# ambonvik/cimba

Measured on NVIDIA H100. Metric: M/M/1 simulated events/sec (FEL pops/s), higher is better.
Workload: dtype f64

## Files before the change

cimba_b200/_lib.py:

```python
from __future__ import annotations

import ctypes as C
from pathlib import Path

import os

LIB_PATH = Path(os.environ.get("CIMBA_B200_LIB") or
                Path(__file__).resolve().parent / "lib" / "libcimba_b200.so")

NO_FIELD = C.c_size_t(-1).value

MODEL_MM1, MODEL_GG1, MODEL_MMC, MODEL_GUARDED, MODEL_PREEMPT, MODEL_BUFFER, MODEL_PRIOQ, MODEL_HOLD, MODEL_TIMERS, MODEL_MM1_RECORDED, MODEL_HARBOR, MODEL_GUARDED_RECORDED, MODEL_BUFFER_RECORDED, MODEL_PRIOQ_RECORDED, MODEL_RESOURCE_RECORDED, MODEL_AWACS = 0, 1, 2, 3, 4, 5, 6, 7, 8, 9, 10, 11, 12, 13, 14, 15
MODEL_RENEGE, MODEL_POOL_RECORDED, MODEL_TUTORIAL1, MODEL_PARK, MODEL_TUTORIAL2, MODEL_USER_BASE, VARIANT_GENERAL, VARIANT_STATIC = 16, 18, 19, 20, 21, 1000, 16, 17
MAP_LANE, MAP_WARP = 1, 32

OK, EINVAL, ENODEVICE, ECUDA, ETRIAL, ENOMEM = 0, -1, -2, -3, -4, -5


class DeviceJob(C.Structure):
    _fields_ = [
        ("model", C.c_int32), ("servers", C.c_int32), ("mapping", C.c_int32), ("variant", C.c_int32),
        ("master_seed", C.c_uint64), ("first_trial", C.c_uint64),
        ("num_trials", C.c_uint64), ("num_objects", C.c_uint64),
        ("arr_mean", C.c_void_p), ("srv_mean", C.c_void_p),
        ("events", C.c_void_p), ("objects", C.c_void_p),
        ("t_end", C.c_void_p), ("sum_wait", C.c_void_p),
        ("status", C.c_void_p), ("max_queue", C.c_void_p), ("counters", C.c_void_p),
        ("workspace", C.c_void_p), ("workspace_bytes", C.c_uint64),
        ("trace_cap", C.c_uint64), ("trace_key", C.c_void_p), ("trace_time", C.c_void_p),
        ("queue_spill_cap", C.c_uint32), ("reserved0", C.c_uint32), ("diag", C.c_void_p),
        ("params", C.POINTER(C.c_double)), ("num_params", C.c_uint32), ("reserved1", C.c_uint32),
    ]


class AwacsTerrain(C.Structure):
    _fields_ = [("map", C.c_void_p), ("cols", C.c_uint32), ("rows", C.c_uint32),
                ("x_scale", C.c_float), ("y_scale", C.c_float),
                ("x_min", C.c_float), ("x_max", C.c_float), ("y_min", C.c_float), ("y_max", C.c_float)]


THREAD_INIT_FUNC = C.CFUNCTYPE(C.c_void_p, C.c_void_p, C.c_uint64)
THREAD_EXIT_FUNC = C.CFUNCTYPE(None, C.c_void_p)


class Experiment(C.Structure):
    _fields_ = [
        ("model", C.c_int32), ("servers", C.c_int32), ("mapping", C.c_int32), ("device", C.c_int32),
        ("variant", C.c_int32), ("queue_spill_cap", C.c_uint32),
        ("master_seed", C.c_uint64), ("first_trial", C.c_uint64), ("num_objects", C.c_uint64),
        ("off_arr_mean", C.c_size_t), ("off_srv_mean", C.c_size_t),
        ("off_obj_cnt", C.c_size_t), ("off_sum_wait", C.c_size_t), ("off_avg_wait", C.c_size_t),
        ("off_events", C.c_size_t), ("off_t_end", C.c_size_t), ("off_status", C.c_size_t),
        ("off_max_queue", C.c_size_t), ("off_counters", C.c_size_t),
        ("params", C.POINTER(C.c_double)), ("num_params", C.c_uint32), ("reserved", C.c_uint32),
    ]


class DataSummaryStruct(C.Structure):
    _fields_ = [
        ("cookie", C.c_uint64), ("count", C.c_uint64),
        ("min", C.c_double), ("max", C.c_double),
        ("m1", C.c_double), ("m2", C.c_double), ("m3", C.c_double), ("m4", C.c_double),
    ]


class WtdSummaryStruct(C.Structure):
    _fields_ = [("base", DataSummaryStruct), ("wsum", C.c_double)]


SYMBOLS = {
    "cimba_b200_workspace_bytes": (C.c_uint64, [C.POINTER(DeviceJob)]),
    "cimba_b200_launch": (C.c_int, [C.POINTER(DeviceJob), C.c_void_p]),
    "cimba_b200_launch_count": (C.c_uint64, []),
    "cimba_b200_summarize": (C.c_int, [C.c_void_p, C.c_void_p, C.c_uint64, C.c_void_p, C.c_void_p]),
    "cimba_b200_run_experiment": (C.c_int, [C.c_void_p, C.c_uint64, C.c_size_t, C.POINTER(Experiment)]),
    "cimba_b200_release_cache": (None, []),
    "cimba_b200_run_experiment_all_gpus": (C.c_int, [C.c_void_p, C.c_uint64, C.c_size_t, C.POINTER(Experiment),
                                                     C.c_int]),
    "cimba_b200_awacs_set_terrain": (C.c_int, [C.POINTER(AwacsTerrain)]),
    "cimba_b200_awacs_upload_terrain": (C.c_int, [C.POINTER(AwacsTerrain)]),
    "cimba_b200_set_thread_hooks": (None, [C.c_void_p, C.c_void_p, C.c_void_p]),
    "cimba_b200_thread_context": (C.c_void_p, []),
    "cimba_b200_datasummary_initialize": (None, [C.POINTER(DataSummaryStruct)]),
    "cimba_b200_datasummary_add": (C.c_uint64, [C.POINTER(DataSummaryStruct), C.c_double]),
    "cimba_b200_datasummary_merge": (C.c_uint64, [C.POINTER(DataSummaryStruct)] * 3),
    "cimba_b200_datasummary_mean": (C.c_double, [C.POINTER(DataSummaryStruct)]),
    "cimba_b200_datasummary_variance": (C.c_double, [C.POINTER(DataSummaryStruct)]),
    "cimba_b200_datasummary_stddev": (C.c_double, [C.POINTER(DataSummaryStruct)]),
    "cimba_b200_datasummary_count": (C.c_uint64, [C.POINTER(DataSummaryStruct)]),
    "cimba_b200_datasummary_max": (C.c_double, [C.POINTER(DataSummaryStruct)]),
    "cimba_b200_datasummary_min": (C.c_double, [C.POINTER(DataSummaryStruct)]),
    "cimba_b200_datasummary_skewness": (C.c_double, [C.POINTER(DataSummaryStruct)]),
    "cimba_b200_datasummary_kurtosis": (C.c_double, [C.POINTER(DataSummaryStruct)]),
    "cimba_b200_datasummary_print": (None, [C.POINTER(DataSummaryStruct), C.c_void_p, C.c_int]),
    "cimba_b200_summarize_weighted": (C.c_int, [C.c_void_p, C.c_void_p, C.c_uint64, C.c_void_p, C.c_void_p]),
    "cimba_b200_merge_weighted_rows": (C.c_int, [C.c_void_p, C.c_uint64, C.c_void_p, C.c_void_p]),
    "cimba_b200_wtdsummary_initialize": (None, [C.POINTER(WtdSummaryStruct)]),
    "cimba_b200_wtdsummary_add": (C.c_uint64, [C.POINTER(WtdSummaryStruct), C.c_double, C.c_double]),
    "cimba_b200_wtdsummary_merge": (C.c_uint64, [C.POINTER(WtdSummaryStruct)] * 3),
    "cimba_b200_wtdsummary_mean": (C.c_double, [C.POINTER(WtdSummaryStruct)]),
    "cimba_b200_wtdsummary_variance": (C.c_double, [C.POINTER(WtdSummaryStruct)]),
    "cimba_b200_wtdsummary_stddev": (C.c_double, [C.POINTER(WtdSummaryStruct)]),
    "cimba_b200_wtdsummary_skewness": (C.c_double, [C.POINTER(WtdSummaryStruct)]),
    "cimba_b200_wtdsummary_kurtosis": (C.c_double, [C.POINTER(WtdSummaryStruct)]),
    "cimba_b200_wtdsummary_print": (None, [C.POINTER(WtdSummaryStruct), C.c_void_p, C.c_int]),
    "cimba_b200_fmix64": (C.c_uint64, [C.c_uint64, C.c_uint64]),
    "cimba_b200_rng_draws": (C.c_int, [C.c_uint64, C.c_int, C.c_double, C.c_double,
                                       C.c_uint64, C.c_void_p, C.c_void_p]),
    "cimba_b200_rng_draws_ex": (C.c_int, [C.c_uint64, C.c_int, C.POINTER(C.c_double), C.c_uint32,
                                          C.c_uint64, C.c_void_p, C.c_void_p]),
    "cimba_b200_alias_create": (C.c_int, [C.c_uint32, C.POINTER(C.c_double), C.POINTER(C.c_uint64),
                                          C.POINTER(C.c_uint32)]),
    "cimba_b200_model_load": (C.c_int, [C.c_char_p]),
    "cimba_b200_model_name": (C.c_char_p, [C.c_int]),
    "cimba_b200_version": (C.c_char_p, []),
    "cimba_b200_last_error": (C.c_char_p, []),
    "cimba_b200_device_count": (C.c_int, []),
}


def load() -> C.CDLL:
    if not LIB_PATH.exists():
        raise ImportError(
            f"{LIB_PATH} is missing: build it with `python -c 'import __graft_entry__ as g; g.build()'` "
            "(nvcc, sm_90a). cimba_b200 has no CPU fallback.")
    lib = C.CDLL(str(LIB_PATH))
    for name, (res, args) in SYMBOLS.items():
        fn = getattr(lib, name)
        fn.restype = res
        fn.argtypes = args
    return lib


lib = load()


class CimbaError(RuntimeError):
    def __init__(self, code: int):
        self.code = code
        msg = lib.cimba_b200_last_error().decode(errors="replace")
        super().__init__(f"cimba_b200 error {code}: {msg}")


def check(code: int) -> None:
    if code != OK:
        raise CimbaError(code)
```

cimba_b200/csrc/capi.cu:

```cuda
#include <atomic>
#include <chrono>
#include <cfloat>
#include <cmath>
#include <cstdio>
#include <cstdlib>
#include <cstring>
#include <deque>
#include <mutex>
#include <string>
#include <thread>
#include <vector>

#include <cuda_runtime.h>

#include "../../include/cimba_b200.h"
#include "engine.cuh"
#include "queue_model.cuh"
#include "mm1_fast.cuh"
#include "mm1_pc.cuh"
#include "gg1_fast.cuh"
#include "pool_model.cuh"
#include "pool_fast.cuh"
#include "guarded_model.cuh"
#include "preempt_model.cuh"
// ... 257 lines not shown
}

template <class Model>
uint64_t engine_workspace(const cimba_b200_device_job *job) { return cmb::workspace_bytes_for<Model>(*job); }

int engine_checks(const cimba_b200_device_job *job, const char *servers_msg)
{
    if (mapping_of(job) != CIMBA_B200_MAP_LANE) return fail(CIMBA_B200_EINVAL, "the general engine runs one trial per lane (CIMBA_B200_MAP_LANE)");
    if (servers_msg != nullptr && job->servers < 1) return fail(CIMBA_B200_EINVAL, servers_msg);
    return check_workspace(job);
}

template <class Model>
int launch_engine(const cimba_b200_device_job *job, cudaStream_t st, const char *what)
{
    return counted(cmb::launch_model<Model>(*job, (unsigned char *)job->workspace, job->workspace_bytes, 0u, st), what);
}

template <class Model> const char *const ENGINE_WHAT = nullptr;
template <> const char *const ENGINE_WHAT<models::MM1> = "trial_kernel<MM1> launch";
template <> const char *const ENGINE_WHAT<models::GG1> = "trial_kernel<GG1> launch";
template <> const char *const ENGINE_WHAT<models::MM1Recorded> = "trial_kernel<MM1Recorded> launch";
template <> const char *const ENGINE_WHAT<models::MMC> = "trial_kernel<MMC> launch";
template <> const char *const ENGINE_WHAT<models::HoldGeneral> = "trial_kernel<HoldGeneral> launch";
template <> const char *const ENGINE_WHAT<models::Renege> = "trial_kernel<Renege> launch";
template <> const char *const ENGINE_WHAT<models::Cheese> = "trial_kernel<Cheese> launch";
template <> const char *const ENGINE_WHAT<models::Tutorial1> = "trial_kernel<Tutorial1> launch";
template <> const char *const ENGINE_WHAT<models::Park> = "trial_kernel<Park> launch";
template <> const char *const ENGINE_WHAT<models::Tutorial2> = "trial_kernel<Tutorial2> launch";

template <class Model>
int engine_launch(const cimba_b200_device_job *job, cudaStream_t st)
{
    if (const int e = engine_checks(job, "servers must be >= 1")) return e;
    return launch_engine<Model>(job, st, ENGINE_WHAT<Model>);
}

template <class Model>
constexpr Route ENGINE{engine_workspace<Model>, engine_launch<Model>};

int harbor_engine_launch(const cimba_b200_device_job *job, cudaStream_t st)
{
    if (const int e = engine_checks(job, "servers must be >= 1")) return e;
    if (job->servers < 3) return fail(CIMBA_B200_EINVAL, "tugs (servers) must be >= 3 for CIMBA_B200_MODEL_HARBOR (a large ship needs 3)");
    return launch_engine<models::HarborGeneral>(job, st, "trial_kernel<HarborGeneral> launch");
}

template <template <class> class ModelT, int NPROC, int NQUEUE, int NEVENT = 0>
uint64_t static_workspace(const cimba_b200_device_job *job) { return cmb::workspace_bytes_static<ModelT, NPROC, NQUEUE, NEVENT>(*job); }

template <template <class> class ModelT, int NPROC, int NQUEUE, int NEVENT = 0>
int static_launch(const cimba_b200_device_job *job, cudaStream_t st)
{
    if (mapping_of(job) != CIMBA_B200_MAP_LANE) return fail(CIMBA_B200_EINVAL, "the static tier runs one trial per lane (CIMBA_B200_MAP_LANE)");
    if (const int e = check_workspace(job)) return e;
    return counted(cmb::launch_static_model<ModelT, NPROC, NQUEUE, NEVENT>(*job, st), "static_trial_kernel launch",
                   job->status != nullptr ? 2 : 1);
}

template <template <class> class ModelT, int NPROC, int NQUEUE, int NEVENT = 0>
constexpr Route STATIC{static_workspace<ModelT, NPROC, NQUEUE, NEVENT>, static_launch<ModelT, NPROC, NQUEUE, NEVENT>};

template <template <class> class ModelT, int NPROC, int NEVENT, uint64_t (*WORKSPACE)(const cimba_b200_device_job *), bool SERVERS>
int static_launch_in(const cimba_b200_device_job *job, cudaStream_t st)
{
    if (mapping_of(job) != CIMBA_B200_MAP_LANE) return fail(CIMBA_B200_EINVAL, "the static tier runs one trial per lane (CIMBA_B200_MAP_LANE)");
    if (SERVERS && job->servers < 1) return fail(CIMBA_B200_EINVAL, "servers must be >= 1");
    if (const int e = check_workspace(job)) return e;
    return counted(cmb::launch_static_trials<ModelT, NPROC, 0, NEVENT>(*job, st), "static_trial_kernel launch",
                   job->status != nullptr ? 2 : 1);
}

template <template <class> class ModelT, int NPROC, int NEVENT, uint64_t (*WORKSPACE)(const cimba_b200_device_job *), bool SERVERS>
constexpr Route STATIC_IN{WORKSPACE, static_launch_in<ModelT, NPROC, NEVENT, WORKSPACE, SERVERS>};

uint64_t queue_rings_bytes(const cimba_b200_device_job *job)
{
    const uint32_t cap = cmb::spill_cap(*job);
    return job->num_trials * (uint64_t)(cap == 0u ? cmb::SPILL_CAP_DEFAULT : cap) * sizeof(double);
}

uint64_t queue_workspace(const cimba_b200_device_job *job) { return cmb::rings_then_arena(queue_rings_bytes(job), repair_arena_bytes(job)); }

int queue_launch(const cimba_b200_device_job *job, cudaStream_t st)
{
    if (const int e = check_workspace(job)) return e;
    const int mapping = mapping_of(job);
    QueueArgs qa = cmb::job_args<QueueArgs>(*job);
    qa.mapping = mapping;
    qa.num_objects = job->num_objects;
    qa.arr_mean = job->arr_mean;
    qa.srv_mean = job->srv_mean;
    qa.counters = job->counters;
    qa.spill = (double *)job->workspace;
    qa.spill_cap = cmb::spill_cap(*job);
    qa.diag = (unsigned long long *)job->diag;
    const uint64_t threads = job->num_trials * (uint64_t)mapping;
    const uint64_t blocks = (threads + QUEUE_BLOCK - 1) / QUEUE_BLOCK;
    if (blocks > 0x7fffffffull) return fail(CIMBA_B200_EINVAL, "too many trials for one launch");
    const dim3 grid((unsigned)blocks);
    const uint64_t rings = queue_rings_bytes(job);
    if (job->model == CIMBA_B200_MODEL_GG1) {
        if (job->variant == 1) return launch_kernel(job, queue_kernel<1, false>, queue_kernel<1, true>, grid, QUEUE_BLOCK, 0, st, qa, "queue_kernel launch");
        return then_repair<models::GG1>(launch_kernel(job, gg1_kernel<false>, gg1_kernel<true>, grid, QUEUE_BLOCK, 0, st, qa, "gg1_kernel launch"),
                                        job, rings, st, "repair pass (G/G/1)");
    }
    if (job->model == CIMBA_B200_MODEL_MM1_RECORDED) {
        if (job->counters == nullptr)
            return fail(CIMBA_B200_EINVAL, "CIMBA_B200_MODEL_MM1_RECORDED writes its cmb_wtdsummary to counters[]");
        const int e = launch_kernel(job, queue_kernel<0, false, true>, queue_kernel<0, true, true>, grid, QUEUE_BLOCK, 0, st, qa,
                                    "queue_kernel (recorded) launch");
        return then_repair<models::MM1Recorded>(e, job, rings, st, "repair pass (M/M/1 with its queue history)");
    }
    if (job->variant == 1) return launch_kernel(job, queue_kernel<0, false>, queue_kernel<0, true>, grid, QUEUE_BLOCK, 0, st, qa, "queue_kernel launch");
    int e;
    if (job->variant == 2) {
        if (mapping != CIMBA_B200_MAP_LANE) return fail(CIMBA_B200_EINVAL, "variant 2 of MODEL_MM1 runs one trial per lane");
        const dim3 pc_grid((unsigned)((job->num_trials + MM1_PC_CONSUMERS - 1) / MM1_PC_CONSUMERS));
        e = launch_kernel(job, mm1_pc_kernel<false>, mm1_pc_kernel<true>, pc_grid, 2 * MM1_PC_CONSUMERS, 0, st, qa, "mm1_kernel launch");
    }
    else {
        e = launch_kernel(job, mm1_kernel<false>, mm1_kernel<true>, grid, QUEUE_BLOCK, 0, st, qa, "mm1_kernel launch");
    }
    return then_repair<models::MM1>(e, job, rings, st, "repair pass (M/M/1)");
}

int mmc_launch(const cimba_b200_device_job *job, cudaStream_t st)
{
    if (job->servers < 1) return fail(CIMBA_B200_EINVAL, "servers must be >= 1 for CIMBA_B200_MODEL_MMC");
    if (mapping_of(job) != CIMBA_B200_MAP_LANE) return fail(CIMBA_B200_EINVAL, "MODEL_MMC supports CIMBA_B200_MAP_LANE only");
    if (const int e = check_workspace(job)) return e;
    PoolArgs pa = cmb::job_args<PoolArgs>(*job);
    pa.servers = job->servers;
    pa.num_objects = job->num_objects;
    pa.arr_mean = job->arr_mean;
    pa.srv_mean = job->srv_mean;
    pa.spill = (double *)job->workspace;
    pa.spill_cap = cmb::spill_cap(*job);
    pa.diag = (unsigned long long *)job->diag;
    const uint64_t blocks = (job->num_trials + POOL_BLOCK - 1) / POOL_BLOCK;
    if (blocks > 0x7fffffffull) return fail(CIMBA_B200_EINVAL, "too many trials for one launch");
    const bool readable = job->variant == 1;
    const int e = launch_kernel(job, readable ? pool_kernel<false> : pool_fast_kernel<false>, readable ? pool_kernel<true> : pool_fast_kernel<true>,
                                dim3((unsigned)blocks), POOL_BLOCK, 0, st, pa, "pool_kernel launch");
    return then_repair<models::MMC>(e, job, queue_rings_bytes(job), st, "repair pass (M/M/c)");
}

bool has_capacity(const cimba_b200_device_job *job)
{
    return job->model != CIMBA_B200_MODEL_TIMERS && job->model != CIMBA_B200_MODEL_RESOURCE_RECORDED;
}

template <bool TRACE>
auto coverage_kernel(int m)
{
    return m == CIMBA_B200_MODEL_RESOURCE_RECORDED ? resource_kernel<TRACE>
         : m == CIMBA_B200_MODEL_TIMERS ? timers_kernel<TRACE>
         : m == CIMBA_B200_MODEL_PRIOQ ? prioq_kernel<TRACE>
         : m == CIMBA_B200_MODEL_BUFFER || m == CIMBA_B200_MODEL_BUFFER_RECORDED ? buffer_kernel<TRACE>
         : m == CIMBA_B200_MODEL_PREEMPT ? preempt_kernel<TRACE>
                                         : guarded_kernel<TRACE>;
}

uint64_t coverage_workspace(const cimba_b200_device_job *job)
{
    return cmb::rings_then_arena(job->num_trials * (uint64_t)sizeof(GeneralState), repair_arena_bytes(job));
}

template <class Model>
int coverage_launch(const cimba_b200_device_job *job, cudaStream_t st)
{
    const int m = job->model;
    if (has_capacity(job) && job->servers < 1) return fail(CIMBA_B200_EINVAL, "capacity (servers) must be >= 1");
    if (mapping_of(job) != CIMBA_B200_MAP_LANE) return fail(CIMBA_B200_EINVAL, "MODEL_GUARDED supports CIMBA_B200_MAP_LANE only");
    if (const int e = check_workspace(job)) return e;
    GuardedArgs ga = cmb::job_args<GuardedArgs>(*job);
    ga.capacity = job->servers;
    ga.duration = job->num_objects;
    ga.put_mean = job->arr_mean;
    ga.get_mean = job->srv_mean;
    ga.counters = job->counters;
    ga.state = (GeneralState *)job->workspace;
    ga.record = (m == CIMBA_B200_MODEL_GUARDED_RECORDED || m == CIMBA_B200_MODEL_BUFFER_RECORDED || m == CIMBA_B200_MODEL_PRIOQ_RECORDED) ? 1u : 0u;
    ga.use_pq = m == CIMBA_B200_MODEL_PRIOQ_RECORDED ? 1u : 0u;
    const uint64_t blocks = (job->num_trials + GUARDED_BLOCK - 1) / GUARDED_BLOCK;
    if (blocks > 0x7fffffffull) return fail(CIMBA_B200_EINVAL, "too many trials for one launch");
    const int e = launch_kernel(job, coverage_kernel<false>(m), coverage_kernel<true>(m), dim3((unsigned)blocks), GUARDED_BLOCK, 0, st, ga,
                                "guarded_kernel launch");
    return then_repair<Model>(e, job, job->num_trials * (uint64_t)sizeof(GeneralState), st, "repair pass");
}

template <class Model>
int coverage_engine_launch(const cimba_b200_device_job *job, cudaStream_t st)
{
    if (const int e = engine_checks(job, has_capacity(job) ? "capacity (servers) must be >= 1" : nullptr)) return e;
    return launch_engine<Model>(job, st, "trial_kernel launch");
}

template <class Model>
const Route *coverage_route(const cimba_b200_device_job *job, int max_servers)
{
    static constexpr Route fast{coverage_workspace, coverage_launch<Model>};
    static constexpr Route engine{engine_workspace<Model>, coverage_engine_launch<Model>};
    return job->variant == CIMBA_B200_VARIANT_GENERAL || job->servers > max_servers ? &engine : &fast;
// ... 107 lines not shown
        const int lanes = job->variant == 2 ? 32 : (job->variant == 4 ? 8 : (job->variant == 3 ? 16 : HOLD_DEFAULT_LANES));
        const void *fn = trace ? (const void *)deep_kernel<true>(lanes) : (const void *)deep_kernel<false>(lanes);
        const uint64_t trials_per_block = (uint64_t)(DEEP_BLOCK / 32) * (uint64_t)(32 / lanes);
        if (const int e = resident_grid(fn, DEEP_BLOCK, 0, 8, (job->num_trials + trials_per_block - 1) / trials_per_block, &blocks)) return e;
        DeepArgs da{};
        da.h = ha;
        da.rows = (uint4 *)job->workspace;
        da.row_entries = deep_row_entries(job->servers);
        return launch_kernel(job, deep_kernel<false>(lanes), deep_kernel<true>(lanes), dim3(blocks), DEEP_BLOCK, 0, st, da, "hold_deep_kernel launch");
    }
    const void *fn = trace ? (const void *)hold_kernel<true> : (const void *)hold_kernel<false>;
    if (const int e = resident_grid(fn, 32, HOLD_SMEM_BYTES, 8, job->num_trials, &blocks)) return e;
    return launch_kernel(job, hold_kernel<false>, hold_kernel<true>, dim3(blocks), 32, HOLD_SMEM_BYTES, st, ha, "hold_kernel launch");
}

uint64_t user_workspace(const cimba_b200_device_job *job) { return user_model(job->model)->workspace_bytes(job); }

int user_launch(const cimba_b200_device_job *job, cudaStream_t st)
{
    if (const int e = check_workspace(job)) return e;
    const UserModel *um = user_model(job->model);
    return counted(um->launch(job, st), um->name.c_str());
}

constexpr Route QUEUE{queue_workspace, queue_launch};
constexpr Route MMC_FAST{queue_workspace, mmc_launch};
constexpr Route HARBOR{harbor_workspace, harbor_launch};
constexpr Route HARBOR_ENGINE{engine_workspace<models::HarborGeneral>, harbor_engine_launch};
constexpr Route AWACS{awacs_workspace, awacs_launch};
constexpr Route HOLD{hold_workspace, hold_launch};
constexpr Route USER{user_workspace, user_launch};

const Route *route(const cimba_b200_device_job *job)
{
    const bool general = job->variant == CIMBA_B200_VARIANT_GENERAL, on_static = job->variant == CIMBA_B200_VARIANT_STATIC;
    switch (job->model) {
    case CIMBA_B200_MODEL_MM1:          return on_static ? &STATIC<models::MM1T, 2, 1> : general ? &ENGINE<models::MM1> : &QUEUE;
    case CIMBA_B200_MODEL_GG1:          return on_static ? &STATIC<models::GG1T, 2, 1> : general ? &ENGINE<models::GG1> : &QUEUE;
    case CIMBA_B200_MODEL_MM1_RECORDED: return on_static ? &STATIC<models::MM1RecordedT, 2, 1> : general ? &ENGINE<models::MM1Recorded> : &QUEUE;
    case CIMBA_B200_MODEL_TUTORIAL1:    return general ? &ENGINE<models::Tutorial1> : &STATIC<models::Tutorial1T, 2, 0, 3>;
    case CIMBA_B200_MODEL_MMC:          return general || job->servers > 14 ? &ENGINE<models::MMC> : &MMC_FAST;
    case CIMBA_B200_MODEL_HOLD:         return general ? &ENGINE<models::HoldGeneral> : &HOLD;
    case CIMBA_B200_MODEL_HARBOR:       return general ? &HARBOR_ENGINE : &HARBOR;
    case CIMBA_B200_MODEL_AWACS:        return &AWACS;
    case CIMBA_B200_MODEL_RENEGE:       return &ENGINE<models::Renege>;
    case CIMBA_B200_MODEL_POOL_RECORDED:
        return on_static ? &STATIC_IN<models::CheeseT, 6, 6, engine_workspace<models::Cheese>, true> : &ENGINE<models::Cheese>;
    case CIMBA_B200_MODEL_PARK:         return &ENGINE<models::Park>;
    case CIMBA_B200_MODEL_TUTORIAL2:
        return on_static ? &STATIC_IN<models::Tutorial2T, 8, 8, engine_workspace<models::Tutorial2>, true> : &ENGINE<models::Tutorial2>;
    case CIMBA_B200_MODEL_GUARDED:
        return on_static ? &STATIC_COVERAGE<models::GuardedQueueT, 7, 1, 2, 16> : coverage_route<models::Guarded<false, false>>(job, 16);
    case CIMBA_B200_MODEL_GUARDED_RECORDED:
        return on_static ? &STATIC_COVERAGE<models::GuardedRecordedQueueT, 7, 1, 2, 16> : coverage_route<models::Guarded<false, true>>(job, 16);
    case CIMBA_B200_MODEL_PRIOQ_RECORDED:
        return on_static ? &STATIC_COVERAGE<models::GuardedPriorityQueueT, 7, 0, 2, 15> : coverage_route<models::Guarded<true, true>>(job, 15);
    case CIMBA_B200_MODEL_PRIOQ:
        return on_static ? &STATIC_COVERAGE<models::QueueAndTideT, 8, 0, 2, 15> : coverage_route<models::QueueAndTide>(job, 15);
    case CIMBA_B200_MODEL_PREEMPT:
        return on_static ? &STATIC_IN<models::PoolFightT, 6, models::POOLFIGHT_SPARE_SLOTS, coverage_workspace, true>
                         : coverage_route<models::PoolFight>(job, INT32_MAX);
    case CIMBA_B200_MODEL_BUFFER:
        return on_static ? &STATIC_IN<models::WorkshopBufferT, 7, models::WORKSHOP_SPARE_SLOTS, coverage_workspace, true>
                         : coverage_route<models::Workshop<false>>(job, INT32_MAX);
    case CIMBA_B200_MODEL_BUFFER_RECORDED:
        return on_static ? &STATIC_IN<models::WorkshopRecordedT, 7, models::WORKSHOP_SPARE_SLOTS, coverage_workspace, true>
                         : coverage_route<models::Workshop<true>>(job, INT32_MAX);
    case CIMBA_B200_MODEL_TIMERS:
        return on_static ? &STATIC_IN<models::FrontDeskT, 8, models::FRONTDESK_SPARE_SLOTS, coverage_workspace, false>
                         : coverage_route<models::FrontDesk>(job, INT32_MAX);
    case CIMBA_B200_MODEL_RESOURCE_RECORDED:
        return on_static ? &STATIC_IN<models::ToolT, 4, 2, coverage_workspace, false> : coverage_route<models::Tool>(job, INT32_MAX);
    }
    return job->model >= CIMBA_B200_MODEL_USER_BASE && user_model(job->model) != nullptr ? &USER : nullptr;
}

}

extern "C" {

const char *cimba_b200_version(void) { return CIMBA_B200_VERSION_STRING; }
const char *cimba_b200_last_error(void) { return g_err; }
uint64_t cimba_b200_launch_count(void) { return g_launches.load(); }
uint64_t cimba_b200_fmix64(uint64_t seed, uint64_t nonce) { return fmix64(seed, nonce); }

int cimba_b200_device_count(void)
{
    int n = 0;
    if (cudaGetDeviceCount(&n) != cudaSuccess) {
        (void)cudaGetLastError();
        return 0;
    }
    return n;
}

uint64_t cimba_b200_workspace_bytes(const cimba_b200_device_job *job)
{
    const Route *r = job != nullptr ? route(job) : nullptr;
    return r != nullptr ? r->workspace(job) : 0u;
}

int cimba_b200_launch(const cimba_b200_device_job *job, void *stream)
{
    if (job == nullptr) return fail(CIMBA_B200_EINVAL, "job is NULL");
    if (job->num_trials == 0u) return fail(CIMBA_B200_EINVAL, "num_trials must be > 0 (src/cimba.c:157)");
    if ((job->arr_mean == nullptr || job->srv_mean == nullptr) && job->model != CIMBA_B200_MODEL_AWACS)
        return fail(CIMBA_B200_EINVAL, "arr_mean/srv_mean device arrays are required");
    if (job->num_objects >= 0xffffffffull) return fail(CIMBA_B200_EINVAL, "num_objects must be < 2^32-1");
    const int mapping = mapping_of(job);
    if (mapping != CIMBA_B200_MAP_LANE && mapping != CIMBA_B200_MAP_WARP)
        return fail(CIMBA_B200_EINVAL, "mapping must be CIMBA_B200_MAP_LANE or CIMBA_B200_MAP_WARP");
    if (job->trace_cap > 0u && (job->trace_key == nullptr || job->trace_time == nullptr))
        return fail(CIMBA_B200_EINVAL, "trace_cap > 0 needs trace_key and trace_time");
    if (cimba_b200_device_count() <= 0) return fail(CIMBA_B200_ENODEVICE, "no CUDA device");
    if (cmb::spill_cap(*job) == 0u)
        return fail(CIMBA_B200_EINVAL, "queue_spill_cap must be 0 (default) or a power of two <= 2^26");
    if (job->num_params > CIMBA_B200_MAX_MODEL_PARAMS || (job->num_params > 0u && job->params == nullptr))
        return fail(CIMBA_B200_EINVAL, "params: at most CIMBA_B200_MAX_MODEL_PARAMS doubles behind a HOST pointer");

    const Route *r = route(job);
    if (r == nullptr)
        return fail(CIMBA_B200_EINVAL, job->model >= CIMBA_B200_MODEL_USER_BASE
                                           ? "unknown model id (cimba_b200_model_load returns the ids of loaded models)" : "unknown model");
    return r->launch(job, (cudaStream_t)stream);
}

namespace {
bool terrain_descriptor_ok(const cimba_b200_awacs_terrain *t)
{
    return t != nullptr && t->map != nullptr && t->cols >= 2u && t->rows >= 2u && t->x_scale > 0.0f && t->y_scale > 0.0f &&
           t->x_min < t->x_max && t->y_min < t->y_max && (uint64_t)t->cols * (uint64_t)t->rows <= 0xffffffffull;
}

int register_terrain(int dev, const cimba_b200_awacs_terrain *t, const float *map, float *owned)
{
    const uint32_t tcols = (t->cols + AWACS_TILE - 1u) >> AWACS_TILE_SHIFT, trows = (t->rows + AWACS_TILE - 1u) >> AWACS_TILE_SHIFT;
    float *tiles = nullptr;
    CUDA_TRY(cudaMalloc(&tiles, (size_t)tcols * trows * sizeof(float)));
    aw_tile_max_kernel<<<dim3(tcols, trows), 256>>>(map, t->cols, t->rows, tiles, tcols);
    g_launches++;
    cudaError_t e = cudaGetLastError();
    if (e == cudaSuccess) e = cudaDeviceSynchronize();
    if (e != cudaSuccess) {
        cudaFree(tiles);
        return cuda_fail(e, "aw_tile_max_kernel");
    }
    std::lock_guard<std::mutex> hold(g_terrain_mu);
    if (g_terrain_tiles[dev] != nullptr) cudaFree(g_terrain_tiles[dev]);
    if (g_terrain_owned[dev] != nullptr && g_terrain_owned[dev] != owned) cudaFree(g_terrain_owned[dev]);
    g_terrain_tiles[dev] = tiles;
    g_terrain_owned[dev] = owned;
    g_terrain[dev] = AwacsTerrain{map, t->cols, t->rows, t->x_scale, t->y_scale, t->x_min, t->x_max, t->y_min, t->y_max,
                                  tiles, tcols, trows};
    g_terrain_set[dev] = true;
    return CIMBA_B200_OK;
}
}

int cimba_b200_awacs_set_terrain(const cimba_b200_awacs_terrain *t)
{
    if (!terrain_descriptor_ok(t)) return fail(CIMBA_B200_EINVAL, "bad terrain descriptor (tutorial/tut_5_1.c:96-108)");
    if (cimba_b200_device_count() <= 0) return fail(CIMBA_B200_ENODEVICE, "no CUDA device");
    int dev = 0;
    CUDA_TRY(cudaGetDevice(&dev));
    if (dev < 0 || dev >= MAX_TERRAIN_DEVICES) return fail(CIMBA_B200_EINVAL, "device index out of range");
    return register_terrain(dev, t, t->map, nullptr);
// ... 605 lines not shown
```

cimba_b200/csrc/mm1_fast.cuh:

```cuda
#pragma once

#include "engine.cuh"
#include "queue_model.cuh"
#include "rng.cuh"

namespace cimba_b200 {

#ifndef MM1_PARK_MASK
#define MM1_PARK_MASK 7u
#endif
#ifndef MM1_COLD_BATCH
#define MM1_COLD_BATCH 4
#endif
#ifndef MM1_STEPS
#define MM1_STEPS 8
#endif

__device__ __forceinline__ void sts_f64(uint32_t addr, double v)
{
    asm volatile("st.shared.f64 [%0], %1;" :: "r"(addr), "d"(v) : "memory");
}

__device__ __forceinline__ double lds_f64(uint32_t addr)
{
    double v;
    asm volatile("ld.shared.f64 %0, [%1];" : "=d"(v) : "r"(addr) : "memory");
    return v;
}

__device__ __forceinline__ uint32_t pack_key(uint32_t counter, uint32_t action)
{
    return (counter << 2) | action;
}

template <bool TRACE>
__global__ void __launch_bounds__(QUEUE_BLOCK)
mm1_kernel(const QueueArgs a)
{
    __shared__ double exp_x[256];
    __shared__ double ring_smem[QUEUE_WINDOW * QUEUE_BLOCK];

    for (unsigned i = threadIdx.x; i < 256u; i += blockDim.x) {
        exp_x[i] = zig::zig_exp_x[i];
    }
    __syncthreads();

    constexpr unsigned FULL = 0xffffffffu;
    constexpr uint32_t WMASK = QUEUE_WINDOW - 1;
    constexpr uint32_t ROW = QUEUE_BLOCK * 8u;
    const double INF = __longlong_as_double(0x7ff0000000000000LL);
    const unsigned lane = threadIdx.x & 31u;
    const uint64_t gtid = (uint64_t)blockIdx.x * blockDim.x + threadIdx.x;
    uint64_t trial;
    bool alive;
    if (a.mapping == 32) {
        trial = gtid >> 5;
        alive = (lane == 0u) && (trial < a.num_trials);
    }
    else {
        trial = gtid;
        alive = trial < a.num_trials;
    }

    Sfc64 rng;
    rng.a = rng.b = rng.c = rng.d = 0u;
    double t_arr = INF, t_srv = INF;
    uint32_t k_arr = 0u, k_srv = 0u;
    uint32_t issued = 0u;
    double now = 0.0, stamp = 0.0, sum_wait = 0.0;
    double arr_mean = 1.0, srv_mean = 1.0;
    uint32_t produced = 0u, served = 0u, dropped = 0u, status = TRIAL_OK, longest = 0u;
    const uint32_t quota = (uint32_t)a.num_objects;
    uint32_t win = (uint32_t)__cvta_generic_to_shared(&ring_smem[threadIdx.x]);
    uint32_t tab = (uint32_t)__cvta_generic_to_shared(&exp_x[0]);
    __shared__ double scratch_smem[QUEUE_BLOCK];
    uint32_t scratch = (uint32_t)__cvta_generic_to_shared(&scratch_smem[threadIdx.x]);
    asm volatile("" : "+r"(win), "+r"(tab), "+r"(scratch));
    double *const spill = (a.spill_cap && alive) ? a.spill + trial * a.spill_cap : nullptr;
    const uint32_t spill_mask = a.spill_cap - 1u;

    uint64_t u_next = 0u;
    double e_next = 0.0;
    uint32_t off_next = 0u;
    uint32_t pops = 0u;
    const auto refill = [&]() {
        u_next = rng.next_imad();
        off_next = imad_hi(imad_lo((uint32_t)u_next, IMAD_K2P24, 0u), IMAD_K2P11, 0u);
        e_next = __dmul_rn(lds_f64(tab + off_next), __ull2double_rn(u_next));
    };

    if (alive) {
        arr_mean = a.arr_mean[trial];
        srv_mean = a.srv_mean[trial];
        rng.seed(fmix64(a.master_seed, a.first_trial + trial));
        t_arr = 0.0; k_arr = pack_key(1u, ACT_START);
        t_srv = 0.0; k_srv = pack_key(2u, ACT_START);
        issued = 2u;
        refill();
    }

    uint32_t flags = alive ? 1u : 0u;
    uint32_t step = 0u;

    const auto event_step = [&]() {
        const bool go0 = flags == 1u;
        const bool first_arr = (t_arr < t_srv) | ((t_arr == t_srv) & (k_arr < k_srv));
        const uint32_t key = first_arr ? k_arr : k_srv;
        const bool go = go0 & (key != 0u);
        if (go0 & (key == 0u)) flags = 0u;
        const bool is_arr = go & first_arr;
        const bool is_srv = go & !first_arr;
        const bool wake = (key & 3u) == ACT_WAKE_TIME;
        if (TRACE) {
            if (go && pops < a.trace_cap) {
                a.trace_key[trial * a.trace_cap + pops] = key >> 2;
                a.trace_time[trial * a.trace_cap + pops] = first_arr ? t_arr : t_srv;
            }
            pops += go ? 1u : 0u;
        }
        if (go) now = first_arr ? t_arr : t_srv;

        const uint32_t p0 = produced, s0 = served;
        const uint32_t q_len = p0 - s0;
        const bool put = is_arr & wake;
        const bool put_far = put & (q_len >= (uint32_t)QUEUE_WINDOW);
        sts_f64((put & !put_far) ? win + (p0 & WMASK) * ROW : scratch, now);
        if (put) produced++;
        if (put & (k_srv == 0u)) {
            issued++;
            t_srv = now;
            k_srv = pack_key(issued, ACT_WAKE_RESOURCE);
        }

        const double new_sum = __dadd_rn(sum_wait, __dsub_rn(now, stamp));
        if (is_srv & wake) sum_wait = new_sum;
        const bool take = is_srv & (q_len != 0u);
        const uint32_t head_slot = win + (s0 & WMASK) * ROW;
        const double head_stamp = lds_f64(head_slot);
        if (take) {
            stamp = head_stamp;
            served++;
        }
        const bool refill_far = take & (q_len > (uint32_t)QUEUE_WINDOW);

        const bool draw = take | (is_arr & (produced < quota));
        const bool hot = off_next <= ZIG_EXP_MAX * 8u;
        const bool push = draw & hot;
        const double when = __dadd_rn(now, __dmul_rn(is_arr ? arr_mean : srv_mean, e_next));
        if (push) issued++;
        const double t_new = push ? when : INF;
        const uint32_t k_new = push ? pack_key(issued, ACT_WAKE_TIME) : 0u;
        if (is_arr) { t_arr = t_new; k_arr = k_new; }
        if (is_srv) { t_srv = t_new; k_srv = k_new; }
        if (draw & !hot) flags = is_arr ? 7u : 3u;
        if (push) refill();

        if (put_far | refill_far) {
            if (refill_far) {
                sts_f64(head_slot, spill[(s0 + QUEUE_WINDOW) & spill_mask]);
            }
            else if (spill != nullptr && q_len - QUEUE_WINDOW <= spill_mask) {
                spill[p0 & spill_mask] = now;
            }
            else {
                status |= TRIAL_ERR_QUEUE_OVERFLOW;
                dropped++;
                served++;
            }
        }
        longest = max(longest, produced - served);
    };

    while (__any_sync(FULL, flags & 1u)) {
#pragma unroll
        for (int i = 0; i < MM1_STEPS; i++) {
            event_step();
        }
        step += MM1_STEPS;
        if ((step & MM1_PARK_MASK) != 0u) {
            continue;
        }
        const unsigned pm = __ballot_sync(FULL, flags & 2u);
        if (pm != 0u) {
            const unsigned am = __ballot_sync(FULL, flags & 1u);
            if (__popc(pm) >= MM1_COLD_BATCH || pm == am) {
                if (flags & 2u) {
                    const bool parked_is_arr = (flags & 4u) != 0u;
                    const double mean = parked_is_arr ? arr_mean : srv_mean;
                    const double at = __dadd_rn(now, __dmul_rn(mean, rng.exp_cold(u_next)));
                    issued++;
                    if (parked_is_arr) { t_arr = at; k_arr = pack_key(issued, ACT_WAKE_TIME); }
                    else               { t_srv = at; k_srv = pack_key(issued, ACT_WAKE_TIME); }
                    flags = 1u;
                    refill();
                }
            }
        }
    }
    if (alive) {
        if (a.events)    a.events[trial] = issued;
        if (a.objects)   a.objects[trial] = served - dropped;
        if (a.t_end)     a.t_end[trial] = now;
        if (a.sum_wait)  a.sum_wait[trial] = sum_wait;
        if (a.status)    a.status[trial] = status | (issued > 0x3ffffff0u ? TRIAL_ERR_KEY_OVERFLOW : 0u);
        if (a.max_queue) a.max_queue[trial] = longest;
    }
    if (a.diag != nullptr && lane == 0u) {
        atomicAdd(a.diag, (unsigned long long)step);
        atomicAdd(a.diag + 1, 1ull);
    }
}

}
```

include/cimba_b200.h:

```cpp
#ifndef CIMBA_B200_H
#define CIMBA_B200_H

#include <stddef.h>
#include <stdint.h>
#include <stdio.h>

#ifdef __cplusplus
extern "C" {
#endif

#define CIMBA_B200_VERSION_STRING "0.1.0"

#define CIMBA_B200_MODEL_MM1 0
#define CIMBA_B200_MODEL_GG1 1
#define CIMBA_B200_MODEL_MMC 2
#define CIMBA_B200_MODEL_GUARDED 3
#define CIMBA_B200_MODEL_PREEMPT 4
#define CIMBA_B200_MODEL_BUFFER 5
#define CIMBA_B200_MODEL_HOLD 7
#define CIMBA_B200_MODEL_PRIOQ 6
#define CIMBA_B200_MODEL_TIMERS 8
#define CIMBA_B200_MODEL_MM1_RECORDED 9
#define CIMBA_B200_MODEL_HARBOR 10
#define CIMBA_B200_MODEL_GUARDED_RECORDED 11
// ... 7 lines not shown

#define CIMBA_B200_MODEL_POOL_RECORDED 18
#define CIMBA_B200_MODEL_TUTORIAL1 19
#define CIMBA_B200_MODEL_PARK 20
#define CIMBA_B200_MODEL_TUTORIAL2 21

#define CIMBA_B200_MODEL_USER_BASE 1000
int cimba_b200_model_load(const char *path_to_model_library);
const char *cimba_b200_model_name(int model_id);

#define CIMBA_B200_VARIANT_GENERAL 16
#define CIMBA_B200_VARIANT_STATIC 17

#define CIMBA_B200_OK         0
#define CIMBA_B200_EINVAL    -1
#define CIMBA_B200_ENODEVICE -2
#define CIMBA_B200_ECUDA     -3
#define CIMBA_B200_ETRIAL    -4
#define CIMBA_B200_ENOMEM    -5

#define CIMBA_B200_TRIAL_QUEUE_OVERFLOW 1u
#define CIMBA_B200_TRIAL_FEL_OVERFLOW   2u
#define CIMBA_B200_TRIAL_KEY_OVERFLOW   4u
#define CIMBA_B200_TRIAL_GUARD_OVERFLOW 8u
#define CIMBA_B200_TRIAL_PROC_OVERFLOW  16u
#define CIMBA_B200_TRIAL_NEGATIVE_HOLD  32u
#define CIMBA_B200_TRIAL_ARENA_EXHAUSTED 64u
#define CIMBA_B200_TRIAL_BAD_ARGUMENT   128u

#define CIMBA_B200_MAP_LANE 1
#define CIMBA_B200_MAP_WARP 32

typedef struct cimba_b200_device_job {
    int32_t  model;
    int32_t  servers;
    int32_t  mapping;
    int32_t  variant;
    uint64_t master_seed;
    uint64_t first_trial;
    uint64_t num_trials;
    uint64_t num_objects;
    const double *arr_mean;
    const double *srv_mean;
    uint64_t *events;
    uint64_t *objects;
    double   *t_end;
    double   *sum_wait;
    uint32_t *status;
    uint32_t *max_queue;
    uint64_t *counters;
    void     *workspace;
    uint64_t  workspace_bytes;
    uint64_t  trace_cap;
    uint64_t *trace_key;
    double   *trace_time;
    uint32_t  queue_spill_cap;
    uint32_t  reserved0;
    uint64_t *diag;
    const double *params;
    uint32_t  num_params;
    uint32_t  reserved1;
} cimba_b200_device_job;
#define CIMBA_B200_MAX_MODEL_PARAMS 16

typedef struct cimba_b200_awacs_terrain {
    const float *map;
    uint32_t cols, rows;
    float x_scale, y_scale;
    float x_min, x_max, y_min, y_max;
} cimba_b200_awacs_terrain;
int cimba_b200_awacs_set_terrain(const cimba_b200_awacs_terrain *terrain);
int cimba_b200_awacs_upload_terrain(const cimba_b200_awacs_terrain *terrain);

#define CIMBA_B200_AWACS_TARGETS 1000
#define CIMBA_B200_AWACS_STRIDE 1024
#define CIMBA_B200_AWACS_STATE_BYTES (CIMBA_B200_AWACS_STRIDE * (7 * 4 + 4 + 4 + 8))

uint64_t cimba_b200_workspace_bytes(const cimba_b200_device_job *job);

int cimba_b200_launch(const cimba_b200_device_job *job, void *stream);

uint64_t cimba_b200_launch_count(void);

int cimba_b200_summarize(const double *sum_wait, const uint64_t *objects,
                         uint64_t num_trials, double *out_summary, void *stream);

int cimba_b200_summarize_weighted(const double *x, const double *w, uint64_t n,
                                  uint64_t *out_row, void *stream);

int cimba_b200_merge_weighted_rows(const uint64_t *rows, uint64_t n, uint64_t *out_row, void *stream);

#define CIMBA_B200_NO_FIELD ((size_t)-1)

typedef struct cimba_b200_experiment {
    int32_t  model;
    int32_t  servers;
    int32_t  mapping;
    int32_t  device;
    int32_t  variant;
    uint32_t queue_spill_cap;
    uint64_t master_seed;
    uint64_t first_trial;
    uint64_t num_objects;
    size_t off_arr_mean;
    size_t off_srv_mean;
    size_t off_obj_cnt;
    size_t off_sum_wait;
    size_t off_avg_wait;
    size_t off_events;
    size_t off_t_end;
    size_t off_status;
    size_t off_max_queue;
    size_t off_counters;
    const double *params;
    uint32_t num_params;
    uint32_t reserved;
} cimba_b200_experiment;

int cimba_b200_run_experiment(void *your_experiment_array,
                              uint64_t num_trials,
                              size_t trial_struct_size,
                              const cimba_b200_experiment *desc);

void cimba_b200_release_cache(void);

int cimba_b200_run_experiment_all_gpus(void *your_experiment_array,
                                       uint64_t num_trials,
                                       size_t trial_struct_size,
                                       const cimba_b200_experiment *desc,
                                       int max_gpus);

typedef void *(cimba_b200_thread_init_func)(void *usrarg, uint64_t tid);
typedef void (cimba_b200_thread_exit_func)(void *thrctx);
void  cimba_b200_set_thread_hooks(cimba_b200_thread_init_func *initfunc, void *usrarg,
                                  cimba_b200_thread_exit_func *exitfunc);
void *cimba_b200_thread_context(void);

typedef struct cimba_b200_datasummary {
    uint64_t cookie;
    uint64_t count;
    double   min, max;
    double   m1, m2, m3, m4;
} cimba_b200_datasummary;

void     cimba_b200_datasummary_initialize(cimba_b200_datasummary *dsp);
uint64_t cimba_b200_datasummary_add(cimba_b200_datasummary *dsp, double y);
uint64_t cimba_b200_datasummary_merge(cimba_b200_datasummary *tgt,
                                      const cimba_b200_datasummary *dsp1,
                                      const cimba_b200_datasummary *dsp2);
double   cimba_b200_datasummary_mean(const cimba_b200_datasummary *dsp);
double   cimba_b200_datasummary_variance(const cimba_b200_datasummary *dsp);
double   cimba_b200_datasummary_stddev(const cimba_b200_datasummary *dsp);
uint64_t cimba_b200_datasummary_count(const cimba_b200_datasummary *dsp);
double   cimba_b200_datasummary_max(const cimba_b200_datasummary *dsp);
double   cimba_b200_datasummary_min(const cimba_b200_datasummary *dsp);
double   cimba_b200_datasummary_skewness(const cimba_b200_datasummary *dsp);
double   cimba_b200_datasummary_kurtosis(const cimba_b200_datasummary *dsp);
void     cimba_b200_datasummary_print(const cimba_b200_datasummary *dsp, FILE *fp, int lead_ins);

typedef struct cimba_b200_wtdsummary {
    cimba_b200_datasummary base;
    double   wsum;
} cimba_b200_wtdsummary;

void     cimba_b200_wtdsummary_initialize(cimba_b200_wtdsummary *wsp);
uint64_t cimba_b200_wtdsummary_add(cimba_b200_wtdsummary *wsp, double x, double w);
// ... 30 lines not shown
```

Before: 148.0 billion.

## Resize M/M/1 shared ring to 48 slots and prefer max shared carveout

Replaces the power-of-two QUEUE_WINDOW ring with a 48-slot ring plus one scratch row, tracked by explicit head/tail byte offsets advanced with a branchless wrap, and folds the separate scratch buffer into the ring allocation. It also sets the preferred shared-memory carveout to maximum for the mm1 kernels so that eight CTAs per SM can be resident, aiming to fit all trials in a single wave. A diagnostic entry point reports resident CTAs per SM. The trade-off is a smaller in-shared-memory window, so deeper queues spill to global memory more often, and the L1 cache gets less capacity.

```diff
diff --git a/cimba_b200/_lib.py b/cimba_b200/_lib.py
--- a/cimba_b200/_lib.py
+++ b/cimba_b200/_lib.py
@@ -72,6 +72,7 @@
     "cimba_b200_workspace_bytes": (C.c_uint64, [C.POINTER(DeviceJob)]),
     "cimba_b200_launch": (C.c_int, [C.POINTER(DeviceJob), C.c_void_p]),
     "cimba_b200_launch_count": (C.c_uint64, []),
+    "cimba_b200_mm1_resident_ctas": (C.c_int, [C.c_int]),
     "cimba_b200_summarize": (C.c_int, [C.c_void_p, C.c_void_p, C.c_uint64, C.c_void_p, C.c_void_p]),
     "cimba_b200_run_experiment": (C.c_int, [C.c_void_p, C.c_uint64, C.c_size_t, C.POINTER(Experiment)]),
     "cimba_b200_release_cache": (None, []),
@@ -119,6 +120,9 @@
 }
 
 
+DIAGNOSTICS = {"cimba_b200_mm1_resident_ctas"}
+
+
 def load() -> C.CDLL:
     if not LIB_PATH.exists():
         raise ImportError(
@@ -126,6 +130,8 @@
             "(nvcc, sm_90a). cimba_b200 has no CPU fallback.")
     lib = C.CDLL(str(LIB_PATH))
     for name, (res, args) in SYMBOLS.items():
+        if name in DIAGNOSTICS and not hasattr(lib, name):
+            continue
         fn = getattr(lib, name)
         fn.restype = res
         fn.argtypes = args
diff --git a/cimba_b200/csrc/capi.cu b/cimba_b200/csrc/capi.cu
--- a/cimba_b200/csrc/capi.cu
+++ b/cimba_b200/csrc/capi.cu
@@ -363,6 +363,19 @@
 
 uint64_t queue_workspace(const cimba_b200_device_job *job) { return cmb::rings_then_arena(queue_rings_bytes(job), repair_arena_bytes(job)); }
 
+int mm1_prefer_shared()
+{
+    static std::atomic<uint64_t> done{0};
+    int dev = 0;
+    CUDA_TRY(cudaGetDevice(&dev));
+    const uint64_t bit = dev < 64 ? 1ull << dev : 0ull;
+    if (bit != 0u && (done.load() & bit) != 0u) return CIMBA_B200_OK;
+    CUDA_TRY(cudaFuncSetAttribute(mm1_kernel<false>, cudaFuncAttributePreferredSharedMemoryCarveout, cudaSharedmemCarveoutMaxShared));
+    CUDA_TRY(cudaFuncSetAttribute(mm1_kernel<true>, cudaFuncAttributePreferredSharedMemoryCarveout, cudaSharedmemCarveoutMaxShared));
+    done.fetch_or(bit);
+    return CIMBA_B200_OK;
+}
+
 int queue_launch(const cimba_b200_device_job *job, cudaStream_t st)
 {
     if (const int e = check_workspace(job)) return e;
@@ -401,6 +414,7 @@
         e = launch_kernel(job, mm1_pc_kernel<false>, mm1_pc_kernel<true>, pc_grid, 2 * MM1_PC_CONSUMERS, 0, st, qa, "mm1_kernel launch");
     }
     else {
+        if (const int c = mm1_prefer_shared()) return c;
         e = launch_kernel(job, mm1_kernel<false>, mm1_kernel<true>, grid, QUEUE_BLOCK, 0, st, qa, "mm1_kernel launch");
     }
     return then_repair<models::MM1>(e, job, rings, st, "repair pass (M/M/1)");
@@ -674,6 +688,15 @@
 const char *cimba_b200_version(void) { return CIMBA_B200_VERSION_STRING; }
 const char *cimba_b200_last_error(void) { return g_err; }
 uint64_t cimba_b200_launch_count(void) { return g_launches.load(); }
+
+int cimba_b200_mm1_resident_ctas(int trace)
+{
+    if (const int e = mm1_prefer_shared()) return e;
+    int per_sm = 0;
+    CUDA_TRY(cudaOccupancyMaxActiveBlocksPerMultiprocessor(&per_sm, trace ? mm1_kernel<true> : mm1_kernel<false>, QUEUE_BLOCK, 0));
+    return per_sm;
+}
+
 uint64_t cimba_b200_fmix64(uint64_t seed, uint64_t nonce) { return fmix64(seed, nonce); }
 
 int cimba_b200_device_count(void)
diff --git a/cimba_b200/csrc/mm1_fast.cuh b/cimba_b200/csrc/mm1_fast.cuh
--- a/cimba_b200/csrc/mm1_fast.cuh
+++ b/cimba_b200/csrc/mm1_fast.cuh
@@ -16,6 +16,10 @@
 #define MM1_STEPS 8
 #endif
 
+constexpr int MM1_WINDOW = 48;
+static_assert(8 * ((MM1_WINDOW + 1) * QUEUE_BLOCK * 8 + 256 * 8 + 1024) <= 228 * 1024,
+              "8 CTAs of mm1_kernel must fit an SM: 65 536 trials in one wave on 132 SMs");
+
 __device__ __forceinline__ void sts_f64(uint32_t addr, double v)
 {
     asm volatile("st.shared.f64 [%0], %1;" :: "r"(addr), "d"(v) : "memory");
@@ -38,7 +42,7 @@
 mm1_kernel(const QueueArgs a)
 {
     __shared__ double exp_x[256];
-    __shared__ double ring_smem[QUEUE_WINDOW * QUEUE_BLOCK];
+    __shared__ double ring_smem[(MM1_WINDOW + 1) * QUEUE_BLOCK];
 
     for (unsigned i = threadIdx.x; i < 256u; i += blockDim.x) {
         exp_x[i] = zig::zig_exp_x[i];
@@ -46,7 +50,6 @@
     __syncthreads();
 
     constexpr unsigned FULL = 0xffffffffu;
-    constexpr uint32_t WMASK = QUEUE_WINDOW - 1;
     constexpr uint32_t ROW = QUEUE_BLOCK * 8u;
     const double INF = __longlong_as_double(0x7ff0000000000000LL);
     const unsigned lane = threadIdx.x & 31u;
@@ -71,11 +74,12 @@
     double arr_mean = 1.0, srv_mean = 1.0;
     uint32_t produced = 0u, served = 0u, dropped = 0u, status = TRIAL_OK, longest = 0u;
     const uint32_t quota = (uint32_t)a.num_objects;
-    uint32_t win = (uint32_t)__cvta_generic_to_shared(&ring_smem[threadIdx.x]);
+    const uint32_t ring = (uint32_t)__cvta_generic_to_shared(&ring_smem[0]);
+    uint32_t tail = threadIdx.x * 8u, head = threadIdx.x * 8u;
+    const uint32_t scratch = MM1_WINDOW * ROW + threadIdx.x * 8u;
+    const auto next_slot = [](uint32_t off) { return min(off + ROW, off - (MM1_WINDOW - 1) * ROW); };
     uint32_t tab = (uint32_t)__cvta_generic_to_shared(&exp_x[0]);
-    __shared__ double scratch_smem[QUEUE_BLOCK];
-    uint32_t scratch = (uint32_t)__cvta_generic_to_shared(&scratch_smem[threadIdx.x]);
-    asm volatile("" : "+r"(win), "+r"(tab), "+r"(scratch));
+    asm volatile("" : "+r"(tab));
     double *const spill = (a.spill_cap && alive) ? a.spill + trial * a.spill_cap : nullptr;
     const uint32_t spill_mask = a.spill_cap - 1u;
 
@@ -123,9 +127,12 @@
         const uint32_t p0 = produced, s0 = served;
         const uint32_t q_len = p0 - s0;
         const bool put = is_arr & wake;
-        const bool put_far = put & (q_len >= (uint32_t)QUEUE_WINDOW);
-        sts_f64((put & !put_far) ? win + (p0 & WMASK) * ROW : scratch, now);
-        if (put) produced++;
+        const bool put_far = put & (q_len >= (uint32_t)MM1_WINDOW);
+        sts_f64(ring + ((put & !put_far) ? tail : scratch), now);
+        if (put) {
+            produced++;
+            tail = next_slot(tail);
+        }
         if (put & (k_srv == 0u)) {
             issued++;
             t_srv = now;
@@ -135,13 +142,14 @@
         const double new_sum = __dadd_rn(sum_wait, __dsub_rn(now, stamp));
         if (is_srv & wake) sum_wait = new_sum;
         const bool take = is_srv & (q_len != 0u);
-        const uint32_t head_slot = win + (s0 & WMASK) * ROW;
-        const double head_stamp = lds_f64(head_slot);
+        const uint32_t h0 = head;
+        const double head_stamp = lds_f64(ring + h0);
         if (take) {
             stamp = head_stamp;
             served++;
-        }
-        const bool refill_far = take & (q_len > (uint32_t)QUEUE_WINDOW);
+            head = next_slot(head);
+        }
+        const bool refill_far = take & (q_len > (uint32_t)MM1_WINDOW);
 
         const bool draw = take | (is_arr & (produced < quota));
         const bool hot = off_next <= ZIG_EXP_MAX * 8u;
@@ -157,15 +165,16 @@
 
         if (put_far | refill_far) {
             if (refill_far) {
-                sts_f64(head_slot, spill[(s0 + QUEUE_WINDOW) & spill_mask]);
-            }
-            else if (spill != nullptr && q_len - QUEUE_WINDOW <= spill_mask) {
+                sts_f64(ring + h0, spill[(s0 + MM1_WINDOW) & spill_mask]);
+            }
+            else if (spill != nullptr && q_len - MM1_WINDOW <= spill_mask) {
                 spill[p0 & spill_mask] = now;
             }
             else {
                 status |= TRIAL_ERR_QUEUE_OVERFLOW;
                 dropped++;
                 served++;
+                head = next_slot(head);
             }
         }
         longest = max(longest, produced - served);
diff --git a/include/cimba_b200.h b/include/cimba_b200.h
--- a/include/cimba_b200.h
+++ b/include/cimba_b200.h
@@ -113,6 +113,8 @@
 
 uint64_t cimba_b200_launch_count(void);
 
+int cimba_b200_mm1_resident_ctas(int trace);
+
 int cimba_b200_summarize(const double *sum_wait, const uint64_t *objects,
                          uint64_t num_trials, double *out_summary, void *stream);
 
```

Measured after the change: 154.8 billion, median of 6. 1.05x the previous value.
